# ucsdarclab/Python-SuPer

Measured on AMD Instinct MI355X. Metric: LM iterations/s (embedded-deformation LM, point-to-plane + ARAP + Rot), higher is better.
Workload: dtype f64; 1 GPU; C2: 200000 surfels / 2000 ED nodes / KNN=4, point-to-plane + ARAP + Rot, 10 LM iterations + Surfels.update per frame; frames_per_gpu=8, streams_per_gpu=1, global_frames=8, parallelism=frames sharded over 1 GPU(s), beta all-gather

## Files before the change

### python-super_amd/csrc/slm_front.hip

```cpp
#include <algorithm>
#include <atomic>
#include <cstdlib>

#include "slm_tile.h"
#include "slm_begin.h"
#include "slm_launch.h"

__device__ __forceinline__ int nd_base(const NDFront& f, int p) {
  return p < f.nv ? 7 * p : f.n1p + 7 * (p - f.nv);
}

__device__ __forceinline__ double* ftile(const FrameDev& fd, const NDFront& f, int r, int c) {
  const size_t t = (size_t)c * f.nt - (size_t)c * (c - 1) / 2 + (size_t)(r - c);
  return fd.ftiles + f.tile_off + t * TILE;
}

__device__ __forceinline__ double* front_entry(const FrameDev& fd, const NDFront& f, int i, int j) {
  return ftile(fd, f, i >> 6, j >> 6) + (i & 63) + (size_t)(j & 63) * NB;
}

__device__ __forceinline__ double* dest_entry(const FrameDev& fd, const NDDest& d, int x, int y) {
  const NDFront& f = fd.fronts[d.front];
  const int rb = nd_base(f, d.prow), cb = nd_base(f, d.pcol);
  return d.transpose ? front_entry(fd, f, rb + y, cb + x) : front_entry(fd, f, rb + x, cb + y);
// ... 224 lines not shown
  const double l2 = lam_a * lam_a;
  if (use_arap && slot < Ke) {
    const int k = frame_in(fd).ed_knn_idx[j * Ke + slot];
    int mult = 0, first = slot;
    for (int s2 = Ke - 1; s2 >= 0; --s2)
      if (frame_in(fd).ed_knn_idx[j * Ke + s2] == k) { ++mult; first = s2; }
    if (k >= 0 && k < J && k != j && first == slot) {
      const NDDest pd = fd.pair_dest[j * Ke + slot];
      const NDFront fp = fd.fronts[pd.front];
      const int prb = nd_base(fp, pd.prow), pcb = nd_base(fp, pd.pcol);
      const bool k_is_row = ((k > j) != (pd.transpose != 0));
      double r[3], Jq[3][4];
      nd_arap_edge(fd, j, k, lam_a, r, Jq);
      int rev = 0;
      for (int s2 = 0; s2 < Ke; ++s2) rev += frame_in(fd).ed_knn_idx[k * Ke + s2] == j;
      const bool reverse = rev > 0;
      const double m = (double)mult;
      double* dst[15];
      double add[15];
#pragma unroll
      for (int c = 0; c < 3; ++c) {
#pragma unroll
        for (int a = 0; a < 4; ++a) {
          add[4 * c + a] = -l2 * Jq[c][a] * m;
          dst[4 * c + a] = k_is_row ? front_entry(fd, fp, prb + a, pcb + 4 + c) : front_entry(fd, fp, prb + 4 + c, pcb + a);
        }
        const bool mine = !reverse || j < k;
        dst[12 + c] = mine ? front_entry(fd, fp, prb + 4 + c, pcb + 4 + c) : nullptr;
        add[12 + c] = -l2 * (double)(mult + rev);
      }
      double cur[15];
#pragma unroll
      for (int e = 0; e < 15; ++e) cur[e] = dst[e] ? *dst[e] : 0.0;
#pragma unroll
      for (int e = 0; e < 15; ++e)
        if (dst[e]) *dst[e] = cur[e] + add[e];
    }
  }
  double acc[28], rh[7];
#pragma unroll
  for (int e = 0; e < 28; ++e) acc[e] = 0.0;
#pragma unroll
  for (int a = 0; a < 7; ++a) rh[a] = 0.0;
  if (use_arap) {
    for (int ie = fd.in_start[j] + slot; ie < fd.in_start[j + 1]; ie += RG_LANES) {
      const int src = fd.in_edge[ie] / Ke;
      if (src == j) continue;
      double r[3], Jq[3][4];
      nd_arap_edge(fd, src, j, lam_a, r, Jq);
#pragma unroll
      for (int a = 0; a < 4; ++a) {
        double gr = 0.0;
#pragma unroll
        for (int c = 0; c < 3; ++c) gr += Jq[c][a] * r[c];
        rh[a] += -lam_a * gr;
#pragma unroll
        for (int b = 0; b <= a; ++b) {
          double q = 0.0;
#pragma unroll
          for (int c = 0; c < 3; ++c) q += Jq[c][a] * Jq[c][b];
          acc[a * (a + 1) / 2 + b] += l2 * q;
        }
      }
#pragma unroll
      for (int c = 0; c < 3; ++c) {
        rh[4 + c] += -lam_a * r[c];
        acc[(4 + c) * (5 + c) / 2 + 4 + c] += l2;
#pragma unroll
        for (int a = 0; a < 4; ++a) acc[(4 + c) * (5 + c) / 2 + a] += l2 * Jq[c][a];
      }
    }
    if (slot < Ke) {
      const int k = frame_in(fd).ed_knn_idx[j * Ke + slot];
      if (k >= 0 && k < J && k != j) {
        double r[3], Jq[3][4];
        nd_arap_edge(fd, j, k, lam_a, r, Jq);
#pragma unroll
        for (int c = 0; c < 3; ++c) {
          rh[4 + c] += lam_a * r[c];
          acc[(4 + c) * (5 + c) / 2 + 4 + c] += l2;
        }
      }
    }
  }
  if (use_rot && slot == 0) {
    double bb[7];
    nd_load_beta(fd.beta, j, bb);
    float q[4];
    const float lam32 = (float)lam_r;
    const float r = nd_rot_residual32(bb, lam32, q);
    float jtj[4][4], jtr[4];
    nd_rot_products32(q, lam32, r, jtj, jtr);
#pragma unroll
    for (int a = 0; a < 4; ++a) {
      rh[a] += (double)jtr[a];
#pragma unroll
      for (int b = 0; b <= a; ++b) acc[a * (a + 1) / 2 + b] += (double)jtj[a][b];
    }
  }
#pragma unroll
  for (int off = 1; off < RG_LANES; off <<= 1) {
#pragma unroll
    for (int e = 0; e < 28; ++e) acc[e] += __shfl_xor(acc[e], off);
#pragma unroll
    for (int a = 0; a < 7; ++a) rh[a] += __shfl_xor(rh[a], off);
  }
  const NDFront fj = fd.fronts[fd.node_front[j]];
  const int bj0 = nd_base(fj, fd.node_pos[j]);
  double* dst[5];
  double add[5], cur[5];
#pragma unroll
  for (int q = 0; q < 5; ++q) {
    const int e = slot + RG_LANES * q;
    dst[q] = nullptr;
    add[q] = 0.0;
    if (e < 28) {
      int a = 0;
      while ((a + 1) * (a + 2) / 2 <= e) ++a;
      const int b = e - a * (a + 1) / 2;
      double v = 0.0;
#pragma unroll
      for (int x = 0; x < 28; ++x) v = (x == e) ? acc[x] : v;
      if (v != 0.0) {
        dst[q] = front_entry(fd, fj, bj0 + a, bj0 + b);
        add[q] = v;
      }
    } else if (e < 35) {
      double v = 0.0;
#pragma unroll
      for (int x = 0; x < 7; ++x) v = (x == e - 28) ? rh[x] : v;
      dst[q] = fd.rhs + 7 * j + (e - 28);
      add[q] = v;
    }
  }
#pragma unroll
  for (int q = 0; q < 5; ++q) cur[q] = dst[q] ? *dst[q] : 0.0;
#pragma unroll
  for (int q = 0; q < 5; ++q)
    if (dst[q]) *dst[q] = cur[q] + add[q];
#pragma unroll
  for (int q = 0; q < 5; ++q) {
    const int e = slot + RG_LANES * q;
    if (e >= 28 && e < 35) fd.fvec[fj.vec_off + 7 * fd.node_pos[j] + (e - 28)] = cur[q] + add[q];
  }
}

__global__ void __launch_bounds__(256) k_front_load_rhs(const FrameDev* __restrict__ frames) {
  const FrameDev& fd = frames[blockIdx.y];
  if (!fd.bound || !fd.nd_ready || fd.st->stopped) return;
  const int e = blockIdx.x * blockDim.x + threadIdx.x;
  if (e >= fd.P) return;
  const int v = e / 7, c = e % 7;
  const NDFront& f = fd.fronts[fd.node_front[v]];
  fd.fvec[f.vec_off + 7 * fd.node_pos[v] + c] = fd.rhs[e];
}

__global__ void __launch_bounds__(256) k_iter_begin_nd(const FrameDev* __restrict__ frames, const int* __restrict__ reuse, int dag_cut) {
  iter_begin_nd_body(frames[blockIdx.y], blockIdx.x, gridDim.x, reuse && reuse[blockIdx.y], dag_cut, false);
}

__global__ void __launch_bounds__(256) k_fpanel(const FrameDev* __restrict__ frames, LevelRef lvl,
                                                 int c, double u_override, WgMap map) {
  extern __shared__ double lds[];
  double *S = PanelLds::S(lds), *M = PanelLds::M(lds), *dinv = PanelLds::dinv(lds), *vec = PanelLds::vec(lds);
  LevelCtx cx;
  if (!level_begin(frames, lvl, c, map, cx)) return;
  const FrameDev& fd = *cx.fd;
  const NDFront& f = *cx.f;
  const int d = cx.unit;
  if (c + d >= f.nt) return;
  const double u = (u_override >= 0.0) ? u_override : fd.st->u;
  const bool stamp = (c == 1 && cx.frame == 0 && cx.front == 0 && d == 1 && lvl.level == fd.n_levels - 1);
  SLM_STAMP(fd, stamp, 0);
  double* At = ftile(fd, f, c + d, c);
  double* yv = fd.fvec + f.vec_off + (size_t)c * NB;
  double4_t a[4];
  panel_column_stage(d, At, yv, ftile(fd, f, c, c), c * NB, f.n1, u, S, vec, a);
  SLM_STAMP(fd, stamp, 1);
  const bool ok = PanelLds::factor(lds, nullptr, nullptr, nullptr, min(4, (f.n1 - c * NB + 15) >> 4));
  SLM_STAMP(fd, stamp, 14);
  if (d == 0 && !ok && threadIdx.x == 0) fd.st->chol_fail = 1;
  panel_column_finish(d, At, yv, fd.flinv + f.linv_off + (size_t)c * TILE, S, M, dinv, vec, a);
  SLM_STAMP(fd, stamp, 15);
}

__global__ void __launch_bounds__(256) k_fpotrf(const FrameDev* __restrict__ frames, LevelRef lvl, int c,
                                                 double u_override) {
  extern __shared__ double lds[];
  double *S = PanelLds::S(lds), *M = PanelLds::M(lds), *dinv = PanelLds::dinv(lds), *vec = PanelLds::vec(lds);
  LevelCtx cx;
  if (!level_begin(frames, lvl, c, cx)) return;
  const FrameDev& fd = *cx.fd;
  const NDFront& f = *cx.f;
  const double u = (u_override >= 0.0) ? u_override : fd.st->u;
  double* yv = fd.fvec + f.vec_off + (size_t)c * NB;
  double4_t a[4];
  panel_column_stage(0, nullptr, yv, ftile(fd, f, c, c), c * NB, f.n1, u, S, vec, a);
  const bool ok = PanelLds::factor(lds, nullptr, nullptr, nullptr, min(4, (f.n1 - c * NB + 15) >> 4));
  if (!ok && threadIdx.x == 0) fd.st->chol_fail = 1;
  panel_column_finish(0, nullptr, yv, fd.flinv + f.linv_off + (size_t)c * TILE, S, M, dinv, vec, a);
}

__global__ void __launch_bounds__(256) k_ftrsm(const FrameDev* __restrict__ frames, LevelRef lvl, int c, WgMap map) {
  __shared__ double Bl[TILE];
  LevelCtx cx;
  if (!level_begin(frames, lvl, c, map, cx)) return;
  const FrameDev& fd = *cx.fd;
  const NDFront& f = *cx.f;
  const int d = cx.unit + 1;
  if (c + d >= f.nt) return;
  double* At = ftile(fd, f, c + d, c);
  tile_product<false, true, false>(fd.flinv + f.linv_off + (size_t)c * TILE, At, At, Bl);
}

__device__ __forceinline__ const NDTileItem* tile_item(const FrameDev* __restrict__ frames, int level, int which, int n_items,
                                                       int at, int n_frames, const FrameDev*& fdp) {
  const int total = n_items * n_frames;
  const int chunk = (total + 7) >> 3;
  const int q = blockIdx.x >> 3;
  const int w_id = (blockIdx.x & 7) * chunk + q;
  if (q >= chunk || w_id >= total) return nullptr;
  const int frame = w_id / n_items, item_idx = w_id - frame * n_items;
  const FrameDev& fd = frames[frame];
  if (!fd.bound || !fd.nd_ready) return nullptr;
  int i0 = at;
  if (at < 0) {
    if (level >= fd.n_levels) return nullptr;
    i0 = fd.item_off[2 * level + which];
    if (item_idx >= fd.item_off[2 * level + which + 1] - i0) return nullptr;
  }
  fdp = &fd;
  return fd.tile_items.get() + i0 + item_idx;
}
__device__ __forceinline__ NDTileItem item_snapshot(const NDTileItem* p) {
  NDTileItem o;
  const int* src = reinterpret_cast<const int*>(p);
  int* dst = reinterpret_cast<int*>(&o);
#pragma unroll
  for (int i = 0; i < (int)(sizeof(NDTileItem) / 4); ++i) dst[i] = __builtin_amdgcn_readfirstlane(src[i]);
  return o;
}
__device__ __forceinline__ double* item_tile(const FrameDev& fd, const NDTileItem& it, int r, int c) {
  const size_t t = (size_t)c * it.nt - (size_t)c * (c - 1) / 2 + (size_t)(r - c);
  return fd.ftiles + (c < it.npt ? it.tile_off : it.f22_base) + t * TILE;
}
__device__ __forceinline__ void pull_maps(const FrameDev& fd, const NDTileItem& it, int2* maps) {
#pragma unroll
  for (int k = 0; k < 2; ++k) {
    if (it.kid[k].front >= 0 && threadIdx.x < 128) {
      const int32_t* pm = fd.pullmap + it.kid[k].pull_off;
      const bool row = threadIdx.x < 64;
      const int c = pm[64 * (row ? it.r : it.c) + (threadIdx.x & 63)];
      int off = 0;
      if (c >= 0) {
        const int t = it.kid[k].npt + (c >> 6);
        off = row ? t * TILE + (c & 63) : (t * it.kid[k].nt - t * (t - 1) / 2 - t) * TILE + (c & 63) * NB;
      }
      maps[128 * k + threadIdx.x] = make_int2(c, off);
    }
  }
}
__device__ __forceinline__ void pull_tile(const FrameDev& fd, const NDTileItem& it, const int2* maps, double4_t acc[4]) {
  const int l = threadIdx.x & 63, w = threadIdx.x >> 6, lr = l & 15, lk = l >> 4;
#pragma unroll
  for (int k = 0; k < 2; ++k) {
    if (it.kid[k].front < 0) continue;
    __builtin_amdgcn_sched_barrier(0);
    double v[16];
    const double* ct = fd.ftiles + it.kid[k].f22_base;
    const int2* mk = maps + 128 * k;
    const int2 rw = mk[16 * w + lr];
#pragma unroll
    for (int ni = 0; ni < 4; ++ni)
#pragma unroll
      for (int rr = 0; rr < 4; ++rr) {
        const int2 cl = mk[64 + 16 * ni + lk + 4 * rr];
        const bool ok = cl.x >= 0 && rw.x >= cl.x;
        const double x = ct[ok ? rw.y + cl.y : 0];
        v[4 * ni + rr] = ok ? x : 0.0;
      }
    __builtin_amdgcn_sched_barrier(0);
#pragma unroll
    for (int ni = 0; ni < 4; ++ni)
#pragma unroll
      for (int rr = 0; rr < 4; ++rr) acc[ni][rr] += v[4 * ni + rr];
    __builtin_amdgcn_sched_barrier(0);
  }
}
__device__ __forceinline__ double pull_vec(const FrameDev& fd, const NDTileItem& it, const int2* maps) {
  double s = 0.0;
  if (threadIdx.x < NB) {
#pragma unroll
    for (int k = 0; k < 2; ++k) {
      if (it.kid[k].front < 0) continue;
      const int ci = maps[128 * k + threadIdx.x].x;
      if (ci >= 0) s += fd.fvec[it.kid[k].vec_boundary + ci];
    }
  }
  return s;
}

__global__ void __launch_bounds__(256, 2) k_fL11(const FrameDev* __restrict__ frames, LevelRef lvl,
                                               double u_override) {
  extern __shared__ double lds[];
  double *S = L11Lds::S(lds), *M = L11Lds::M(lds);
  double* Bl = L11Lds::Bl(lds);
  double* vec = L11Lds::vec(lds);
  double* part = L11Lds::vec2(lds);
  LevelCtx cx;
  if (!level_begin(frames, lvl, 0, cx)) return;
  const FrameDev& fd = *cx.fd;
  const NDFront& f = *cx.f;
  const double u = (u_override >= 0.0) ? u_override : fd.st->u;
  double* vecs = fd.fvec + f.vec_off;
  const int w = threadIdx.x >> 6, l = threadIdx.x & 63, lr = l & 15, lk = l >> 4;

  for (int c = 0; c < f.npt; ++c) {
    double rhs_c = 0.0;
    {
      double v[16];
      tile_to_regs(ftile(fd, f, c, c), v);
      if (threadIdx.x < NB) rhs_c = vecs[(size_t)c * NB + threadIdx.x];
#pragma unroll
      for (int t = 0; t < 16; ++t) {
        const int e = threadIdx.x + 256 * t;
        const int i = e % NB, k = e / NB;
        double x = (i >= k) ? v[t] : 0.0;
        if (i == k) x = (c * NB + i < f.n1) ? x + u : 1.0;
        S[i + k * LD] = x;
      }
    }
    __syncthreads();
    const bool ok = L11Lds::factor(lds, nullptr, nullptr, nullptr, min(4, (f.n1 - c * NB + 15) >> 4));
    if (!ok && threadIdx.x == 0) fd.st->chol_fail = 1;
    if (threadIdx.x < NB) vec[threadIdx.x] = rhs_c;
    __syncthreads();
    {
      commit_pivot(M, vec, fd.flinv + f.linv_off + (size_t)c * TILE, part);
      __syncthreads();
      if (threadIdx.x < NB) {
        vec[threadIdx.x] = part[threadIdx.x];
        vecs[(size_t)c * NB + threadIdx.x] = part[threadIdx.x];
      }
      __syncthreads();
    }
    for (int r = c + 1; r < f.npt; ++r) {
      double* At = ftile(fd, f, r, c);
      double areg[16];
      load_a_frags(At, areg);
      double4_t acc[4];
      zero_acc(acc);
      tile_ABt_regs<false, true>(areg, M, acc);
      store_c_frags(At, acc);
      const double sacc = sum_row_lanes(acc_dot_vec(acc, vec, 0.0));
      if (lk == 0) vecs[(size_t)r * NB + 16 * w + lr] -= sacc;
    }
    __syncthreads();
    for (int sc = c + 1; sc < f.npt; ++sc) {
      double breg[16];
      tile_to_regs(ftile(fd, f, sc, c), breg);
      __syncthreads();
      regs_to_lds(Bl, breg);
      __syncthreads();
      for (int r = sc; r < f.npt; ++r) {
        double* Ct = ftile(fd, f, r, sc);
        double areg[16];
        load_a_frags(ftile(fd, f, r, c), areg);
        double4_t acc[4];
        load_c_frags(Ct, acc);
        if (r == sc) tile_ABt_regs_trim<true>(areg, Bl, acc, 4, w + 1);
        else tile_ABt_regs<true>(areg, Bl, acc);
        store_c_frags(Ct, acc);
      }
    }
    __syncthreads();
  }
}

__global__ void __launch_bounds__(256, 3) k_fL21(const FrameDev* __restrict__ frames, LevelRef lvl, WgMap map) {
  __shared__ double Bl[TILE];
  __shared__ double yv[NB];
  LevelCtx cx;
  if (!level_begin(frames, lvl, 0, map, cx)) return;
  const FrameDev& fd = *cx.fd;
  const NDFront& f = *cx.f;
  const int r = f.npt + cx.unit;
  if (r >= f.nt) return;
  const int w = threadIdx.x >> 6, l = threadIdx.x & 63, lr = l & 15, lk = l >> 4;
  double* vecs = fd.fvec + f.vec_off;
  const bool wave_on = 16 * w < min(NB, 7 * f.nb - NB * cx.unit);
  double rhs_acc = 0.0;
  for (int c = 0; c < f.npt; ++c) {
    {
      const int ncol = min(NB, f.n1 - NB * c);
      const int nblk = (ncol + 15) >> 4;
      double* At = ftile(fd, f, r, c);
      double4_t acc[4];
      if (wave_on) load_c_frags(At, acc);
      else zero_acc(acc);
      for (int cp = 0; cp < c; ++cp) {
        const double* Lt = ftile(fd, f, c, cp);
        double breg[16], xreg[16];
        tile_to_regs(Lt, breg);
        if (wave_on) load_a_frags(ftile(fd, f, r, cp), xreg);
        __syncthreads();
        regs_to_lds(Bl, breg);
        __syncthreads();
        if (wave_on) tile_ABt_regs_trim<true>(xreg, Bl, acc, 4, nblk);
      }
      {
        const double* linv = fd.flinv + f.linv_off + (size_t)c * TILE;
        double breg[16];
        tile_to_regs(linv, breg);
        __syncthreads();
        regs_to_lds(Bl, breg);
        if (threadIdx.x < NB) yv[threadIdx.x] = vecs[(size_t)c * NB + threadIdx.x];
        __syncthreads();
        double areg[16];
#pragma unroll
        for (int ni = 0; ni < 4; ++ni)
#pragma unroll
          for (int rr = 0; rr < 4; ++rr) areg[4 * ni + rr] = acc[ni][rr];
        double4_t xa[4];
        zero_acc(xa);
        if (wave_on) {
          tile_ABt_regs_trim<false, true>(areg, Bl, xa, nblk, nblk);
          store_c_frags_nblk(At, xa, nblk);
        }
        rhs_acc = acc_dot_vec(xa, yv, rhs_acc);
      }
    }
  }
  rhs_acc = sum_row_lanes(rhs_acc);
  if (lk == 0 && wave_on) vecs[(size_t)r * NB + 16 * w + lr] -= rhs_acc;
}

__global__ void __launch_bounds__(256) k_ftrail(const FrameDev* __restrict__ frames, LevelRef lvl,
                                                 int c, int mcap, int bcap, int ntile_cap, WgMap map) {
  __shared__ double Bl[TILE];
  LevelCtx cx;
  if (!level_begin(frames, lvl, c, map, cx)) return;
  const FrameDev& fd = *cx.fd;
  const NDFront& f = *cx.f;
  const int m = f.nt - 1 - c;
  int t = cx.unit;
  if (t < ntile_cap) {
    int db = 1;
    while (db <= bcap && t >= mcap - db + 1) {
      t -= mcap - db + 1;
      ++db;
    }
    const int da = db + t;
    if (da > m || c + db >= f.npt) return;
    tile_product<true, false, true>(ftile(fd, f, c + db, c), ftile(fd, f, c + da, c), ftile(fd, f, c + da, c + db), Bl);
  } else {
    const int db = t - ntile_cap + 1;
    if (db > m) return;
    __shared__ double y[NB];
    __shared__ double part[4 * NB];
    double* vecs = fd.fvec + f.vec_off;
    trail_rhs(ftile(fd, f, c + db, c), vecs + (size_t)c * NB, vecs + (size_t)(c + db) * NB, y, part);
  }
}

__global__ void __launch_bounds__(256) k_fpull(const FrameDev* __restrict__ frames, int level, int n_items, int items_at,
                                                int n_frames) {
  __shared__ int2 maps[256];
  const FrameDev* fdp;
  const NDTileItem* itp = tile_item(frames, level, 1, n_items, items_at, n_frames, fdp);
  if (!itp) return;
  const FrameDev& fd = *fdp;
  const NDTileItem it = item_snapshot(itp);
  const int w = threadIdx.x >> 6;
  const int vrow = it.r < it.npt ? min(NB, it.n1 - NB * it.r) : min(NB, it.n2 - NB * (it.r - it.npt));
  const int nblk = (min(NB, it.n1 - NB * it.c) + 15) >> 4;
  const bool wave_on = 16 * w < vrow;
  pull_maps(fd, it, maps);
  double* T = item_tile(fd, it, it.r, it.c);
  const bool pure = __builtin_amdgcn_readfirstlane((int)fd.tile_kind[it.pad0]) != 0;
  double4_t acc[4];
  zero_acc(acc);
  if (wave_on && !pure) load_c_frags_nblk(T, acc, nblk);
  __syncthreads();
  if (wave_on) pull_tile(fd, it, maps, acc);
  if (pure) store_c_frags(T, acc);
  else if (wave_on) store_c_frags_nblk(T, acc, nblk);
  if (it.r == it.c) {
    const double v = pull_vec(fd, it, maps);
    if (threadIdx.x < NB && v != 0.0) fd.fvec[it.vec_off + (size_t)it.c * NB + threadIdx.x] += v;
  }
}

__global__ void __launch_bounds__(256, 3) k_fschur(const FrameDev* __restrict__ frames, int level, int n_items,
                                                 int items_at, int n_frames) {
  __shared__ __attribute__((aligned(16))) double Bl[TILE];
  __shared__ int2 maps[256];
  const FrameDev* fdp;
  const NDTileItem* itp = tile_item(frames, level, 0, n_items, items_at, n_frames, fdp);
  if (!itp) return;
  const FrameDev& fd = *fdp;
  const NDTileItem& it = *itp;
  const int r = it.r, sc = it.c, tr = r - it.npt, tc = sc - it.npt;
  const int l = threadIdx.x & 63, w = threadIdx.x >> 6, lr = l & 15, lk = l >> 4;
  const int vrow = min(NB, it.n2 - NB * tr), vcol = min(NB, it.n2 - NB * tc);
  const bool wave_on = 16 * w < vrow;
  const int nblk = (tr == tc) ? min((vcol + 15) >> 4, w + 1) : (vcol + 15) >> 4;
  const bool kids = it.kid[0].front >= 0 || it.kid[1].front >= 0;
  pull_maps(fd, it, maps);
  typedef double dvec2 __attribute__((ext_vector_type(2)));
  dvec2 breg[4];
  double areg[16], acur[16];
  if (it.npt > 0) {
    const dvec2* Ls = reinterpret_cast<const dvec2*>(item_tile(fd, it, sc, 0));
#pragma unroll
    for (int e = 0; e < 4; ++e) breg[e] = Ls[threadIdx.x + 256 * e];
    if (wave_on) load_a_frags(item_tile(fd, it, r, 0), areg);
  }
  double4_t acc[4];
  zero_acc(acc);
  __syncthreads();
  if (kids) pull_tile(fd, it, maps, acc);
  for (int c = 0; c < it.npt; ++c) {
    const dvec2* Ls = reinterpret_cast<const dvec2*>(item_tile(fd, it, sc, c));
    dvec2* Bl2 = reinterpret_cast<dvec2*>(Bl);
    const int ksteps = min(16, (it.n1 - NB * c + 3) >> 2);
#pragma unroll
    for (int e = 0; e < 4; ++e) Bl2[threadIdx.x + 256 * e] = breg[e];
#pragma unroll
    for (int e = 0; e < 16; ++e) acur[e] = areg[e];
    if (ksteps > 8) {
#pragma unroll
      for (int e = 0; e < 4; ++e) breg[e] = Ls[TILE / 4 + threadIdx.x + 256 * e];
    }
    if (c + 1 < it.npt && wave_on) load_a_frags(item_tile(fd, it, r, c + 1), areg);
    __syncthreads();
    if (wave_on) {
#pragma unroll
      for (int ks = 0; ks < 8; ++ks) {
        if (ks < ksteps) {
          const double av = -acur[ks];
#pragma unroll
          for (int ni = 0; ni < 4; ++ni)
            if (ni < nblk)
              acc[ni] = __builtin_amdgcn_mfma_f64_16x16x4f64(Bl[(16 * ni + lr) + (4 * ks + lk) * LD], av, acc[ni], 0, 0, 0);
        }
      }
    }
    if (ksteps > 8) {
#pragma unroll
      for (int e = 0; e < 4; ++e) Bl2[TILE / 4 + threadIdx.x + 256 * e] = breg[e];
    }
    if (c + 1 < it.npt) {
      const dvec2* Ln = reinterpret_cast<const dvec2*>(item_tile(fd, it, sc, c + 1));
#pragma unroll
      for (int e = 0; e < 4; ++e) breg[e] = Ln[threadIdx.x + 256 * e];
    }
    __syncthreads();
    if (wave_on) {
#pragma unroll
      for (int ks = 8; ks < 16; ++ks) {
        if (ks < ksteps) {
          const double av = -acur[ks];
#pragma unroll
          for (int ni = 0; ni < 4; ++ni)
            if (ni < nblk)
              acc[ni] = __builtin_amdgcn_mfma_f64_16x16x4f64(Bl[(16 * ni + lr) + (4 * ks + lk) * LD], av, acc[ni], 0, 0, 0);
        }
      }
    }
  }
  if (wave_on) store_c_frags_nblk(item_tile(fd, it, r, sc), acc, nblk);
  if (tr == tc && kids) {
    const double v = pull_vec(fd, it, maps);
    if (threadIdx.x < NB && v != 0.0) fd.fvec[it.vec_off + (size_t)r * NB + threadIdx.x] += v;
  }
}

__global__ void __launch_bounds__(256) k_fback_prep(const FrameDev* __restrict__ frames, LevelRef lvl) {
  extern __shared__ double xb[];
  LevelCtx cx;
  if (!level_begin(frames, lvl, blockIdx.x, cx)) return;
  const FrameDev& fd = *cx.fd;
  const NDFront& f = *cx.f;
  const int c = cx.unit;
  if (f.nb == 0) return;
  const int* nodes = fd.nd_nodes + f.nodes_off + f.nv;
  for (int i = threadIdx.x; i < f.n2p; i += blockDim.x)
    xb[i] = (i < 7 * f.nb) ? fd.delta[7 * nodes[i / 7] + i % 7] : 0.0;
  __syncthreads();
  double acc = 0.0;
  for (int r = f.npt; r < f.nt; ++r) acc = tile_t_vec_lanes(ftile(fd, f, r, c), xb + (size_t)(r - f.npt) * NB, acc);
  acc = sum_col_lanes(acc);
  if ((threadIdx.x & 3) == 0) fd.fvec[f.vec_off + (size_t)c * NB + (threadIdx.x >> 2)] -= acc;
}

__global__ void __launch_bounds__(256) k_fbacksub(const FrameDev* __restrict__ frames, LevelRef lvl,
                                                   int step) {
  LevelCtx cx;
  if (!level_begin(frames, lvl, step, cx)) return;
  const FrameDev& fd = *cx.fd;
  const NDFront& f = *cx.f;
  const int c = f.npt - 1 - step;
  const int d = cx.unit;
  if (d > c) return;
  __shared__ double y[NB];
  __shared__ double x[NB];
  __shared__ double part[4 * NB];
  double* vecs = fd.fvec + f.vec_off;
  backsub_x(fd.flinv + f.linv_off + (size_t)c * TILE, vecs + (size_t)c * NB, y, x, part);
  if (d == 0) {
    if (threadIdx.x < NB) {
      const int i = c * NB + threadIdx.x;
      if (i < f.n1) {
        const int node = fd.nd_nodes[f.nodes_off + i / 7];
        fd.delta[7 * node + i % 7] = x[threadIdx.x];
      }
    }
  } else {
    backsub_update(ftile(fd, f, c, c - d), x, vecs + (size_t)(c - d) * NB);
  }
}

void launch_pair_reduce(const FrameDev* fr, int n_frames, int max_blocks, hipStream_t st) {
  if (max_blocks <= 0) return;
  hipLaunchKernelGGL(k_pair_reduce, dim3((max_blocks + 3) / 4, n_frames), dim3(256), 0, st, fr);
}

void launch_pair_scatter(const FrameDev* fr, int n_frames, int max_blocks, hipStream_t st) {
  if (max_blocks <= 0) return;
  hipLaunchKernelGGL(k_pair_scatter, dim3((max_blocks + 3) / 4, n_frames), dim3(256), 0, st, fr);
}

void launch_front_assemble(const FrameDev* fr, int n_frames, int max_blocks, hipStream_t st) {
  if (max_blocks <= 0) return;
  hipLaunchKernelGGL(k_front_assemble, dim3((max_blocks + 3) / 4, n_frames), dim3(256), 0, st, fr);
}

void launch_reg_grad_nd(const FrameDev* fr, int n_frames, int maxJ, int use_arap, double lam_a,
                        int use_rot, double lam_r, hipStream_t st) {
  if (maxJ <= 0 || (!use_arap && !use_rot)) return;
  hipLaunchKernelGGL(k_reg_grad_nd, dim3((maxJ * RG_LANES + 255) / 256, n_frames), dim3(256), 0, st, fr, use_arap,
                     lam_a, use_rot, lam_r);
}

void launch_front_load_rhs(const FrameDev* fr, int n_frames, int maxP, hipStream_t st) {
  hipLaunchKernelGGL(k_front_load_rhs, dim3((maxP + 255) / 256, n_frames), dim3(256), 0, st, fr);
}

void launch_iter_begin_nd(const FrameDev* fr, int n_frames, hipStream_t st, const int* reuse, int dag_cut) {
  hipLaunchKernelGGL(k_iter_begin_nd, dim3(1024, n_frames), dim3(256), 0, st, fr, reuse, dag_cut);
}

bool ensure_dynamic_lds(const void* kernel, size_t bytes) {
  static std::atomic<const void*> done[64][8];
  int dev = 0;
  (void)hipGetDevice(&dev);
  const bool tracked = dev >= 0 && dev < 64;
  if (tracked)
    for (auto& slot : done[dev])
      if (slot.load(std::memory_order_acquire) == kernel) return true;
  if (hipFuncSetAttribute(kernel, hipFuncAttributeMaxDynamicSharedMemorySize, (int)bytes) != hipSuccess) return false;
  if (tracked)
    for (auto& slot : done[dev]) {
      const void* seen = nullptr;
      if (slot.compare_exchange_strong(seen, kernel, std::memory_order_acq_rel) || seen == kernel) break;
    }
  return true;
}

void launch_front_levels(const FrameDev* fr, int n_frames, const NDLevelSched* lv, int n_levels, int l_factor_end,
// ... 76 lines not shown
```

### python-super_amd/csrc/slm_tile.h

```cpp
#pragma once
#include "slm_common.h"

typedef double double4_t __attribute__((ext_vector_type(4)));

__device__ __forceinline__ void trace_put(long long* trc, int k, long long v) {
  typedef __attribute__((address_space(1))) long long gll;
  *((gll*)(trc + k)) = v;
}

#define NB SLM_NB
#define TILE (NB * NB)

#define LD NB

__device__ __forceinline__ void wave_sync() {
  __builtin_amdgcn_fence(__ATOMIC_RELEASE, "wavefront");
  __builtin_amdgcn_wave_barrier();
  __builtin_amdgcn_fence(__ATOMIC_ACQUIRE, "wavefront");
}

template <bool NEG>
__device__ __forceinline__ double4_t blk_mma(double4_t acc, const double* X, int xs_m, int xs_p,
                                             const double* Y, int ys_p, int ys_n) {
  const int l = threadIdx.x & 63, lr = l & 15, lk = l >> 4;
// ... 185 lines not shown
  wave_sync();
}
__device__ __forceinline__ void blk_trail(double* S, int ib, int jb, int kb) {
  double* Cb = S + ib * 16 + jb * 16 * LD;
  double4_t acc = blk_load(Cb, 1, LD);
  acc = blk_mma<true>(acc, S + ib * 16 + kb * 16 * LD, 1, LD, S + jb * 16 + kb * 16 * LD, LD, 1);
  blk_store(Cb, 1, LD, acc);
}

#define SLM_MAIL_DOUBLES 2560
#define SLM_MAIL_EMPTY 0x7FF8DEADBEEF0001ll
__device__ __forceinline__ void publish_blocks16(const double* S, const double* dinv, int kb, double* g_mail) {
  typedef __attribute__((address_space(1))) double gdbl;
  const int l = threadIdx.x & 63;
#pragma unroll
  for (int j = 0; j < 4; ++j) {
    const int e = l + 64 * j;
    __hip_atomic_store((gdbl*)(g_mail + kb * 256 + e), dinv[kb * 256 + e], __ATOMIC_RELAXED, __HIP_MEMORY_SCOPE_AGENT);
  }
  for (int t = 0; t < kb; ++t)
#pragma unroll
    for (int j = 0; j < 4; ++j) {
      const int e = l + 64 * j, i = e & 15, k = e >> 4;
      __hip_atomic_store((gdbl*)(g_mail + (4 + kb * (kb - 1) / 2 + t) * 256 + e), S[(16 * kb + i) + (16 * t + k) * LD],
                         __ATOMIC_RELAXED, __HIP_MEMORY_SCOPE_AGENT);
    }
}

__device__ __forceinline__ bool factor_inverse64p(double* S, double* M, double* dinv, double* wt, double* xch,
                                                  int* s_ok, int* pf, double* g_mail = nullptr, int* g_early = nullptr,
                                                  long long* trc = nullptr, int nblk = 4, double* la_blk = nullptr,
                                                  const double* la_part = nullptr, double* la_sum = nullptr) {
#define FTRC(k) do { if (trc && threadIdx.x == 0) trace_put(trc, (k), wall_clock64()); } while (0)
  const int w = threadIdx.x >> 6;
  const double4_t z4 = {0.0, 0.0, 0.0, 0.0};
  if (threadIdx.x < 16) pf[threadIdx.x] = 0;
  if (threadIdx.x == 0) *s_ok = 1;
  if (!la_blk) __syncthreads();
  double* Wscr = wt + (w > 0 ? w - 1 : 0) * 256;
  int* vpf = pf;
#pragma unroll 1
  for (int kb = 0; kb < 4; ++kb) {
    FTRC(3 * kb);
    if (w == 0) {
      if (kb < nblk) {
        const bool staged = kb == 0 && la_blk;
        const bool ok = diag16(staged ? la_blk : S + kb * 16 * (LD + 1), dinv + kb * 256, xch, staged ? 16 : LD);
        if (!ok && (threadIdx.x & 63) == 0) *s_ok = 0;
      } else {
        const int l = threadIdx.x & 63;
#pragma unroll
        for (int j = 0; j < 4; ++j) {
          const int e = l + 64 * j;
          dinv[kb * 256 + e] = ((e & 15) == (e >> 4)) ? 1.0 : 0.0;
        }
        wave_sync();
      }
      FTRC(3 * kb + 1);
    } else if (kb == 0) {
      for (int e = threadIdx.x - 64; e < 6 * 256; e += 192) {
        const int b = e >> 8, ib = b < 3 ? 0 : (b < 5 ? 1 : 2), jb = b < 3 ? b + 1 : (b < 5 ? b - 1 : 3);
        M[(16 * ib + (e & 15)) + (16 * jb + ((e >> 4) & 15)) * LD] = 0.0;
      }
    } else if (kb == 1) {
      lds_wait_all(vpf + 0, 3);
      if (w == 1) { blk_trail(S, 2, 1, 0); blk_trail(S, 3, 2, 0); }
      else if (w == 2) { blk_trail(S, 2, 2, 0); blk_trail(S, 3, 3, 0); }
      else blk_trail(S, 3, 1, 0);
    } else if (kb == 2) {
      lds_wait_all(vpf + 4, 2);
      if (w == 1) blk_trail(S, 3, 2, 1);
      else if (w == 2) blk_trail(S, 3, 3, 1);
      else {
        const double4_t t = blk_LM(z4, S + 16, dinv, true);
        blk_neg_dinv_store(M + 16, dinv + 256, Wscr, t);
      }
    } else {
      lds_wait_all(vpf + 8, 1);
      if (w == 3) {
        double4_t t = blk_LM(z4, S + 32 + 16 * LD, dinv + 256, true);
        blk_neg_dinv_store(M + 32 + 16 * LD, dinv + 512, Wscr, t);
        t = blk_LM(z4, S + 48 + 16 * LD, dinv + 256, true);
        t = blk_LM(t, S + 48 + 32 * LD, M + 32 + 16 * LD, false);
        blk_store(Wscr, 1, 16, t);
      } else if (w == 1) {
        double4_t t = blk_LM(z4, S + 32, dinv, true);
        t = blk_LM(t, S + 32 + 16 * LD, M + 16, false);
        blk_neg_dinv_store(M + 32, dinv + 512, Wscr, t);
        t = blk_LM(z4, S + 48, dinv, true);
        t = blk_LM(t, S + 48 + 16 * LD, M + 16, false);
        t = blk_LM(t, S + 48 + 32 * LD, M + 32, false);
        blk_store(Wscr, 1, 16, t);
      } else {
        const double4_t t = blk_LM(z4, S + 48 + 32 * LD, dinv + 512, true);
        blk_store(Wscr, 1, 16, t);
      }
      wave_sync();
    }
    if (kb == 0 && g_early) asm volatile("s_waitcnt vmcnt(0)" ::: "memory");
    __syncthreads();
    FTRC(3 * kb + 2);
    if (kb == 0 && la_part && threadIdx.x < NB)
      *la_sum = la_part[threadIdx.x] + la_part[NB + threadIdx.x] + la_part[2 * NB + threadIdx.x] + la_part[3 * NB + threadIdx.x];
    if (kb == 3) break;
    if (g_mail && w == (kb == 0 ? 3 : 2)) publish_blocks16(S, dinv, kb, g_mail);
    if (kb == 0 && g_early && threadIdx.x == 128)
      __hip_atomic_store((__attribute__((address_space(1))) int*)g_early, 1, __ATOMIC_RELAXED, __HIP_MEMORY_SCOPE_AGENT);
    if (w < 3 - kb) {
      const int ib = kb + 1 + w;
      double* Xb = S + ib * 16 + kb * 16 * LD;
      double4_t acc = blk_mma<false>(z4, Xb, 1, LD, dinv + kb * 256, 16, 1);
      blk_store(Xb, 1, LD, acc);
      wave_sync();
      lds_signal(vpf + 4 * kb + w);
    }
    if (w == 0) {
      blk_trail(S, kb + 1, kb + 1, kb);
      wave_sync();
    }
  }
  if (w >= 1) {
    const int j = (w == 1) ? 0 : (w == 2 ? 2 : 1);
    double4_t m2 = blk_mma<true>(z4, dinv + 768, 1, 16, Wscr, 1, 16);
    blk_store(M + 48 + j * 16 * LD, 1, LD, m2);
  } else {
    if (g_mail) publish_blocks16(S, dinv, 3, g_mail);
    for (int e = threadIdx.x; e < 1024; e += 64) {
      const int b = e >> 8, i = e & 15, k = (e >> 4) & 15;
      M[(16 * b + i) + (16 * b + k) * LD] = dinv[b * 256 + i + 16 * k];
    }
  }
  __syncthreads();
  FTRC(12);
#undef FTRC
  return *s_ok != 0;
}

template <int NVEC, int NINT = 32>
struct TileLds {
  static_assert(NVEC >= 2, "the exchange buffer is the last two vectors");
  enum : int {
    DINV_DOUBLES = 4 * 256, WT_DOUBLES = 3 * 256,
    S_AT = 0, M_AT = TILE, DINV_AT = 2 * TILE, WT_AT = DINV_AT + DINV_DOUBLES, VEC_AT = WT_AT + WT_DOUBLES,
    XCH_AT = VEC_AT + (NVEC - 2) * NB, INT_AT = VEC_AT + NVEC * NB, DOUBLES = INT_AT + NINT / 2
  };
  enum : int {
    INT_OK = 0, INT_TASK = 1, INT_ABORT = 2, INT_CNT = 3, INT_VOTES = 4, INT_PF = 8
  };
  static_assert(NINT % 2 == 0 && INT_PF + 16 <= NINT, "the int block and pf lie inside the size");
  static_assert(256 * sizeof(int2) <= DINV_DOUBLES * sizeof(double), "maps (256 int2) fit in dinv");
  static_assert(4 * NB <= WT_DOUBLES, "part (4 NB) fits in wt");
  static __device__ __forceinline__ double* S(double* lds) { return lds + S_AT; }
  static __device__ __forceinline__ double* M(double* lds) { return lds + M_AT; }
  static __device__ __forceinline__ double* Bl(double* lds) { return S(lds); }
  static __device__ __forceinline__ double* dinv(double* lds) { return lds + DINV_AT; }
  static __device__ __forceinline__ int2* maps(double* lds) { return reinterpret_cast<int2*>(dinv(lds)); }
  static __device__ __forceinline__ double* wt(double* lds) { return lds + WT_AT; }
  static __device__ __forceinline__ double* part(double* lds) { return wt(lds); }
  static __device__ __forceinline__ double* vec(double* lds) { return lds + VEC_AT; }
  static __device__ __forceinline__ double* vec2(double* lds) { return vec(lds) + NB; }
  static __device__ __forceinline__ double* xch(double* lds) { return lds + XCH_AT; }
  static __device__ __forceinline__ int* ints(double* lds) { return reinterpret_cast<int*>(lds + INT_AT); }
  static __device__ __forceinline__ int* s_ok(double* lds) { return ints(lds) + INT_OK; }
  static __device__ __forceinline__ int* s_task(double* lds) { return ints(lds) + INT_TASK; }
  static __device__ __forceinline__ int* s_abort(double* lds) { return ints(lds) + INT_ABORT; }
  static __device__ __forceinline__ int* s_cnt(double* lds) { return ints(lds) + INT_CNT; }
  static __device__ __forceinline__ int* votes(double* lds) { return ints(lds) + INT_VOTES; }
  static __device__ __forceinline__ int* pf(double* lds) { return ints(lds) + INT_PF; }
  static __device__ __forceinline__ bool factor(double* lds, double* g_mail = nullptr, int* g_early = nullptr, long long* trc = nullptr,
                                                int nblk = 4, bool look_ahead = false, double* la_sum = nullptr) {
    return factor_inverse64p(S(lds), M(lds), dinv(lds), wt(lds), xch(lds), s_ok(lds), pf(lds), g_mail, g_early, trc, nblk,
                             look_ahead ? dinv(lds) + 256 : nullptr, look_ahead ? wt(lds) : nullptr, la_sum);
  }
};
typedef TileLds<3> PanelLds;
typedef TileLds<2> L11Lds;
typedef TileLds<2, 48> DagLds;
#define PANEL_LDS_DOUBLES (PanelLds::DOUBLES)
#define L11_LDS_DOUBLES (L11Lds::DOUBLES)
#define DAG_LDS_DOUBLES (DagLds::DOUBLES)
static_assert(PANEL_LDS_DOUBLES * 8 == 81536 && L11_LDS_DOUBLES * 8 == 81024 && DAG_LDS_DOUBLES * 8 == 81088,
              "launch sizes: two workgroups per CU (160 KB of LDS) were measured with these");

__device__ __forceinline__ void load_a_frags(const double* __restrict__ A, double areg[16]) {
  const int l = threadIdx.x & 63, w = threadIdx.x >> 6, lr = l & 15, lk = l >> 4;
#pragma unroll
  for (int ks = 0; ks < 16; ++ks) areg[ks] = A[(16 * w + lr) + (size_t)(4 * ks + lk) * NB];
}

__device__ __forceinline__ void load_c_frags(const double* __restrict__ Cg, double4_t acc[4]) {
  const int l = threadIdx.x & 63, w = threadIdx.x >> 6, lr = l & 15, lk = l >> 4;
#pragma unroll
  for (int ni = 0; ni < 4; ++ni)
#pragma unroll
    for (int r = 0; r < 4; ++r) acc[ni][r] = Cg[(16 * w + lr) + (size_t)(16 * ni + lk + 4 * r) * NB];
}

template <bool NEGATE, bool LOWER_B = false>
__device__ __forceinline__ void tile_ABt_regs(const double areg[16], const double* Bl,
                                              double4_t acc[4]) {
  const int l = threadIdx.x & 63, lr = l & 15, lk = l >> 4;
#pragma unroll
  for (int ks = 0; ks < 16; ++ks) {
    const double a = NEGATE ? -areg[ks] : areg[ks];
#pragma unroll
    for (int ni = LOWER_B ? (ks >> 2) : 0; ni < 4; ++ni) {
      const double b = Bl[(16 * ni + lr) + (4 * ks + lk) * LD];
      acc[ni] = __builtin_amdgcn_mfma_f64_16x16x4f64(b, a, acc[ni], 0, 0, 0);
    }
    if ((ks & 3) == 3) __builtin_amdgcn_sched_barrier(0);
  }
}

template <bool NEGATE, int NBLK, bool LOWER_B>
__device__ __forceinline__ void tile_ABt_regs_nblk(const double areg[16], const double* Bl, double4_t acc[4], int kblk) {
  const int l = threadIdx.x & 63, lr = l & 15, lk = l >> 4;
#pragma unroll
  for (int kb = 0; kb < 4; ++kb) {
    if (kb < kblk) {
#pragma unroll
      for (int k4 = 0; k4 < 4; ++k4) {
        const int ks = 4 * kb + k4;
        const double a = NEGATE ? -areg[ks] : areg[ks];
#pragma unroll
        for (int ni = LOWER_B ? kb : 0; ni < NBLK; ++ni) {
          const double b = Bl[(16 * ni + lr) + (4 * ks + lk) * LD];
          acc[ni] = __builtin_amdgcn_mfma_f64_16x16x4f64(b, a, acc[ni], 0, 0, 0);
        }
      }
    }
    __builtin_amdgcn_sched_barrier(0);
  }
}
template <bool NEGATE, bool LOWER_B = false>
__device__ __forceinline__ void tile_ABt_regs_trim(const double areg[16], const double* Bl, double4_t acc[4], int kblk,
                                                   int nblk) {
  switch (nblk) {
    case 1: tile_ABt_regs_nblk<NEGATE, 1, LOWER_B>(areg, Bl, acc, kblk); break;
    case 2: tile_ABt_regs_nblk<NEGATE, 2, LOWER_B>(areg, Bl, acc, kblk); break;
    case 3: tile_ABt_regs_nblk<NEGATE, 3, LOWER_B>(areg, Bl, acc, kblk); break;
    default: tile_ABt_regs_nblk<NEGATE, 4, LOWER_B>(areg, Bl, acc, kblk); break;
  }
}

__device__ __forceinline__ void store_c_frags(double* __restrict__ Cg, const double4_t acc[4]) {
  const int l = threadIdx.x & 63, w = threadIdx.x >> 6, lr = l & 15, lk = l >> 4;
#pragma unroll
  for (int ni = 0; ni < 4; ++ni)
#pragma unroll
    for (int r = 0; r < 4; ++r) Cg[(16 * w + lr) + (size_t)(16 * ni + lk + 4 * r) * NB] = acc[ni][r];
}

__device__ __forceinline__ void trsm_rows16(const double* S, const double* dinv, double4_t a[4]) {
  const int l = threadIdx.x & 63, lr = l & 15, lk = l >> 4;
#pragma unroll
  for (int kb = 0; kb < 4; ++kb) {
    double4_t acc = a[kb];
#pragma unroll
    for (int t = 0; t < kb; ++t) {
#pragma unroll
      for (int ks = 0; ks < 4; ++ks) {
        const double y = S[(16 * kb + lr) + (16 * t + 4 * ks + lk) * LD];
        acc = __builtin_amdgcn_mfma_f64_16x16x4f64(y, -a[t][ks], acc, 0, 0, 0);
      }
    }
    double4_t x = {0.0, 0.0, 0.0, 0.0};
#pragma unroll
    for (int ks = 0; ks < 4; ++ks) {
      const double y = dinv[kb * 256 + lr + 16 * (4 * ks + lk)];
      x = __builtin_amdgcn_mfma_f64_16x16x4f64(y, acc[ks], x, 0, 0, 0);
    }
    a[kb] = x;
  }
}

__device__ __forceinline__ double damped_lower(double x, int i, int k, int row0, int n_rows, double u) {
  x = (i >= k) ? x : 0.0;
  if (i == k) x = (row0 + i < n_rows) ? x + u : 1.0;
  return x;
}

__device__ __forceinline__ void tile_to_regs(const double* src, double v[16]) {
#pragma unroll
  for (int e = 0; e < 16; ++e) v[e] = src[threadIdx.x + 256 * e];
}
__device__ __forceinline__ void regs_to_lds(double* Bl, const double v[16]) {
#pragma unroll
  for (int e = 0; e < 16; ++e) Bl[threadIdx.x + 256 * e] = v[e];
}
__device__ __forceinline__ void regs_to_diag_tile(const double v[16], int row0, int n_rows, double u, double* S) {
#pragma unroll
  for (int t = 0; t < 16; ++t) {
    const int e = threadIdx.x + 256 * t;
    const int i = e % NB, k = e / NB;
    S[i + k * LD] = damped_lower(v[t], i, k, row0, n_rows, u);
  }
}
__device__ __forceinline__ void stage_diag_tile(const double* src, int row0, int n_rows, double u, double* S) {
  double v[16];
  tile_to_regs(src, v);
  regs_to_diag_tile(v, row0, n_rows, u, S);
}

__device__ __forceinline__ void commit_pivot(const double* M, const double* vec, double* linv, double* y_out) {
  for (int e = threadIdx.x; e < TILE; e += blockDim.x) linv[e] = M[e];
  if (threadIdx.x < NB) {
    const int i = threadIdx.x;
    double acc = 0.0;
    for (int k = 0; k <= i; ++k) acc += M[i + k * LD] * vec[k];
    y_out[i] = acc;
  }
}

__device__ __forceinline__ void zero_acc(double4_t acc[4]) {
#pragma unroll
  for (int ni = 0; ni < 4; ++ni) acc[ni] = double4_t{0.0, 0.0, 0.0, 0.0};
}
__device__ __forceinline__ void load_c_frags_nblk(const double* Cg, double4_t acc[4], int nblk) {
  const int l = threadIdx.x & 63, w = threadIdx.x >> 6, lr = l & 15, lk = l >> 4;
#pragma unroll
  for (int ni = 0; ni < 4; ++ni)
    if (ni < nblk) {
#pragma unroll
      for (int rr = 0; rr < 4; ++rr) acc[ni][rr] = Cg[(16 * w + lr) + (size_t)(16 * ni + lk + 4 * rr) * NB];
    }
}
__device__ __forceinline__ void store_c_frags_nblk(double* Cg, const double4_t acc[4], int nblk) {
  const int l = threadIdx.x & 63, w = threadIdx.x >> 6, lr = l & 15, lk = l >> 4;
#pragma unroll
  for (int ni = 0; ni < 4; ++ni)
    if (ni < nblk) {
#pragma unroll
      for (int rr = 0; rr < 4; ++rr) Cg[(16 * w + lr) + (size_t)(16 * ni + lk + 4 * rr) * NB] = acc[ni][rr];
    }
}

__device__ __forceinline__ double acc_dot_vec(const double4_t acc[4], const double* y, double s) {
  const int lk = (threadIdx.x & 63) >> 4;
#pragma unroll
  for (int ni = 0; ni < 4; ++ni)
#pragma unroll
    for (int rr = 0; rr < 4; ++rr) s += acc[ni][rr] * y[16 * ni + lk + 4 * rr];
  return s;
}
__device__ __forceinline__ double sum_row_lanes(double s) {
  s += __shfl_xor(s, 16, 64);
  s += __shfl_xor(s, 32, 64);
  return s;
}

template <bool TRANSPOSED>
__device__ __forceinline__ double tile_vec_quarters(const double* T, const double* v, double* part) {
  const int i = threadIdx.x & 63, q = threadIdx.x >> 6;
  double acc = 0.0;
#pragma unroll
  for (int k = 16 * q; k < 16 * q + 16; ++k) acc += (TRANSPOSED ? T[k + i * NB] : T[i + k * NB]) * v[k];
  part[q * NB + i] = acc;
  __syncthreads();
  return threadIdx.x < NB ? part[i] + part[NB + i] + part[2 * NB + i] + part[3 * NB + i] : 0.0;
}
__device__ __forceinline__ double tile_t_vec_lanes(const double* T, const double* x, double acc) {
  const int n = threadIdx.x >> 2, q = threadIdx.x & 3;
#pragma unroll
  for (int mrow = 16 * q; mrow < 16 * q + 16; ++mrow) acc += T[mrow + n * NB] * x[mrow];
  return acc;
}
__device__ __forceinline__ double sum_col_lanes(double acc) {
  acc += __shfl_xor(acc, 1, 64);
  acc += __shfl_xor(acc, 2, 64);
  return acc;
}

__device__ __forceinline__ void panel_column_stage(int d, const double* At, const double* yv, const double* diag, int row0,
                                                   int n_rows, double u, double* S, double* vec, double4_t a[4]) {
  if (d > 0) load_c_frags(At, a);
  else if (threadIdx.x < NB) vec[threadIdx.x] = yv[threadIdx.x];
  stage_diag_tile(diag, row0, n_rows, u, S);
  __syncthreads();
}
__device__ __forceinline__ void panel_column_finish(int d, double* At, double* yv, double* linv, const double* S, const double* M,
                                                    const double* dinv, const double* vec, double4_t a[4]) {
  if (d == 0) {
    commit_pivot(M, vec, linv, yv);
  } else {
    trsm_rows16(S, dinv, a);
    store_c_frags(At, a);
  }
}

template <bool NEGATE, bool LOWER_B, bool ACCUMULATE>
__device__ __forceinline__ void tile_product(const double* Bt, const double* At, double* Ct, double* Bl) {
  double breg[16];
  tile_to_regs(Bt, breg);
  double areg[16];
  load_a_frags(At, areg);
  double4_t acc[4];
  if (ACCUMULATE) load_c_frags(Ct, acc);
  regs_to_lds(Bl, breg);
  __syncthreads();
  if (!ACCUMULATE) zero_acc(acc);
  tile_ABt_regs<NEGATE, LOWER_B>(areg, Bl, acc);
  store_c_frags(Ct, acc);
}

__device__ __forceinline__ void trail_rhs(const double* Ls, const double* yc, double* bs, double* y, double* part) {
  if (threadIdx.x < NB) y[threadIdx.x] = yc[threadIdx.x];
  __syncthreads();
  const double s = tile_vec_quarters<false>(Ls, y, part);
  if (threadIdx.x < NB) bs[threadIdx.x] -= s;
}

__device__ __forceinline__ void backsub_x(const double* linv, const double* yc, double* y, double* x, double* part) {
  if (threadIdx.x < NB) y[threadIdx.x] = yc[threadIdx.x];
  __syncthreads();
  const double s = tile_vec_quarters<true>(linv, y, part);
  if (threadIdx.x < NB) x[threadIdx.x] = s;
  __syncthreads();
}
__device__ __forceinline__ void backsub_update(const double* Lt, const double* x, double* yr) {
  const double acc = sum_col_lanes(tile_t_vec_lanes(Lt, x, 0.0));
  if ((threadIdx.x & 3) == 0) yr[threadIdx.x >> 2] -= acc;
}
```

Before: 3399 LM it/s.

## Pipeline fL11 panel: prefetch A tile, reverse panel loop, keep first panel in LDS

Reworks the blocked Cholesky loop in k_fL11. It prefetches the last panel tile's A fragments during the pivot commit and walks the panel update in reverse so that prefetch is used first. The first off-diagonal panel tile result is written straight to LDS, which skips reloading it from global memory in the trailing update. The next column's RHS is loaded early, and an asm barrier on the LDS pointer is added to control compiler scheduling. The cost is more register pressure, and the reordered stores and loads need care to stay correct.

```diff
diff --git a/python-super_amd/csrc/slm_front.hip b/python-super_amd/csrc/slm_front.hip
--- a/python-super_amd/csrc/slm_front.hip
+++ b/python-super_amd/csrc/slm_front.hip
@@ -550,11 +550,7 @@
 
 __global__ void __launch_bounds__(256, 2) k_fL11(const FrameDev* __restrict__ frames, LevelRef lvl,
                                                double u_override) {
-  extern __shared__ double lds[];
-  double *S = L11Lds::S(lds), *M = L11Lds::M(lds);
-  double* Bl = L11Lds::Bl(lds);
-  double* vec = L11Lds::vec(lds);
-  double* part = L11Lds::vec2(lds);
+  extern __shared__ double lds0[];
   LevelCtx cx;
   if (!level_begin(frames, lvl, 0, cx)) return;
   const FrameDev& fd = *cx.fd;
@@ -562,25 +558,45 @@
   const double u = (u_override >= 0.0) ? u_override : fd.st->u;
   double* vecs = fd.fvec + f.vec_off;
   const int w = threadIdx.x >> 6, l = threadIdx.x & 63, lr = l & 15, lk = l >> 4;
-
-  for (int c = 0; c < f.npt; ++c) {
-    double rhs_c = 0.0;
+  const int npt = f.npt, n1 = f.n1;
+  auto lds_here = [&]() {
+    int zero = 0;
+    asm volatile("" : "+s"(zero));
+    return lds0 + zero;
+  };
+
+  double rhs_c = 0.0;
+  for (int c = 0; c < npt; ++c) {
+    const bool more = c + 1 < npt;
+    double* lds = lds_here();
     {
+      double* S = L11Lds::S(lds);
       double v[16];
       tile_to_regs(ftile(fd, f, c, c), v);
-      if (threadIdx.x < NB) rhs_c = vecs[(size_t)c * NB + threadIdx.x];
+      if (c == 0 && threadIdx.x < NB) rhs_c = vecs[threadIdx.x];
 #pragma unroll
       for (int t = 0; t < 16; ++t) {
         const int e = threadIdx.x + 256 * t;
         const int i = e % NB, k = e / NB;
         double x = (i >= k) ? v[t] : 0.0;
-        if (i == k) x = (c * NB + i < f.n1) ? x + u : 1.0;
+        if (i == k) x = (c * NB + i < n1) ? x + u : 1.0;
         S[i + k * LD] = x;
       }
     }
     __syncthreads();
-    const bool ok = L11Lds::factor(lds, nullptr, nullptr, nullptr, min(4, (f.n1 - c * NB + 15) >> 4));
+    const bool ok = factor_inverse64p(L11Lds::S(lds), L11Lds::M(lds), L11Lds::dinv(lds), L11Lds::wt(lds), L11Lds::xch(lds), L11Lds::s_ok(lds),
+                                      L11Lds::pf(lds), nullptr, nullptr, nullptr, min(4, (n1 - c * NB + 15) >> 4));
     if (!ok && threadIdx.x == 0) fd.st->chol_fail = 1;
+    lds = lds_here();
+    double* M = L11Lds::M(lds);
+    double* Bl = L11Lds::Bl(lds);
+    double* vec = L11Lds::vec(lds);
+    double* part = L11Lds::vec2(lds);
+    double areg[16];
+    if (more) {
+      load_a_frags(ftile(fd, f, npt - 1, c), areg);
+      __builtin_amdgcn_sched_barrier(0);
+    }
     if (threadIdx.x < NB) vec[threadIdx.x] = rhs_c;
     __syncthreads();
     {
@@ -592,28 +608,33 @@
       }
       __syncthreads();
     }
-    for (int r = c + 1; r < f.npt; ++r) {
+    for (int r = npt - 1; r > c; --r) {
       double* At = ftile(fd, f, r, c);
-      double areg[16];
-      load_a_frags(At, areg);
+      if (r < npt - 1) load_a_frags(At, areg);
       double4_t acc[4];
       zero_acc(acc);
       tile_ABt_regs<false, true>(areg, M, acc);
+      const double sacc = sum_row_lanes(acc_dot_vec(acc, vec, 0.0));
       store_c_frags(At, acc);
-      const double sacc = sum_row_lanes(acc_dot_vec(acc, vec, 0.0));
+      if (r == c + 1) acc_to_lds(Bl, acc);
       if (lk == 0) vecs[(size_t)r * NB + 16 * w + lr] -= sacc;
     }
     __syncthreads();
-    for (int sc = c + 1; sc < f.npt; ++sc) {
-      double breg[16];
-      tile_to_regs(ftile(fd, f, sc, c), breg);
-      __syncthreads();
-      regs_to_lds(Bl, breg);
-      __syncthreads();
-      for (int r = sc; r < f.npt; ++r) {
+    if (more && threadIdx.x < NB) rhs_c = vecs[(size_t)(c + 1) * NB + threadIdx.x];
+    lds = lds_here();
+    Bl = L11Lds::Bl(lds);
+    for (int sc = c + 1; sc < npt; ++sc) {
+      if (sc > c + 1) {
+        double breg[16];
+        tile_to_regs(ftile(fd, f, sc, c), breg);
+        __syncthreads();
+        regs_to_lds(Bl, breg);
+        __syncthreads();
+      }
+      for (int r = sc; r < npt; ++r) {
         double* Ct = ftile(fd, f, r, sc);
-        double areg[16];
-        load_a_frags(ftile(fd, f, r, c), areg);
+        if (r == c + 1) load_a_frags(Bl, areg);
+        else load_a_frags(ftile(fd, f, r, c), areg);
         double4_t acc[4];
         load_c_frags(Ct, acc);
         if (r == sc) tile_ABt_regs_trim<true>(areg, Bl, acc, 4, w + 1);
diff --git a/python-super_amd/csrc/slm_tile.h b/python-super_amd/csrc/slm_tile.h
--- a/python-super_amd/csrc/slm_tile.h
+++ b/python-super_amd/csrc/slm_tile.h
@@ -511,6 +511,15 @@
   regs_to_diag_tile(v, row0, n_rows, u, S);
 }
 
+__device__ __forceinline__ void acc_to_lds(double* Bl, const double4_t acc[4]) {
+  const int l = threadIdx.x & 63, w = threadIdx.x >> 6, lr = l & 15, lk = l >> 4;
+  double* mine = Bl + (16 * w + lr) + lk * LD;
+#pragma unroll
+  for (int ni = 0; ni < 4; ++ni)
+#pragma unroll
+    for (int rr = 0; rr < 4; ++rr) mine[(16 * ni + 4 * rr) * LD] = acc[ni][rr];
+}
+
 __device__ __forceinline__ void commit_pivot(const double* M, const double* vec, double* linv, double* y_out) {
   for (int e = threadIdx.x; e < TILE; e += blockDim.x) linv[e] = M[e];
   if (threadIdx.x < NB) {
```

Measured after the change: 3438 LM it/s, median of 6. +1.1%, better.
